# jonnydubowsky/hbbft

Measured on AMD Instinct MI355X. Metric: BLS12-381 share verifies/sec (node) at N=256; crypto ms per HB epoch, higher is better.
Workload: dtype i32 (Fq as 14 signed 28-bit digits, R = 2^392, in the share check; 12 x u32 limbs elsewhere)

## Files before the change

hbbft_amd/csrc/g1d.hpp:

```cpp
#pragma once
#include "g2d.hpp"

namespace hbx {

struct g1jd {
  fqd x, y, z;
};

HBX_HD g1jd g1d_dbl(const g1jd& p) {
  const fqd A = fqd_sqr(p.x);
  const fqd B = fqd_sqr(p.y);
  const fqd C = fqd_sqr(B);
  const fqd D = fqd_dbl(fqd_relax(fqd_sub(fqd_sub(fqd_sqr(fqd_add(p.x, B)), A), C)));
  const fqd E = fqd_relax(fqd_add(fqd_dbl(A), A));
  const fqd F = fqd_sqr(E);
  const fqd X3 = fqd_relax(fqd_sub(F, fqd_dbl(D)));
  const fqd C8 = fqd_dbl(fqd_dbl(fqd_dbl(C)));
  const fqd Y3 = fqd_relax(fqd_sub(fqd_mul(E, fqd_sub(D, X3)), C8));
  const fqd Z3 = fqd_relax(fqd_dbl(fqd_mul(p.y, p.z)));
  return g1jd{X3, Y3, Z3};
}

HBX_HD g1jd g1d_add_mixed(const g1jd& p, const fqd& qx, const fqd& qy) {
  const fqd one = fqd_const(FQD_ONE);
// ... 45 lines not shown
#pragma unroll 1
  for (int i = 2; i < 16; i++) tab[i] = g1d_add_mixed(tab[i - 1], px, py);
  const uint32_t top = k4[3] >> 28;
  g1jd acc = tab[top];
  bool ai = top == 0;
#pragma unroll 1
  for (int w = 30; w >= 0; w--) {
    const uint32_t nib = (k4[w >> 3] >> ((w & 7) * 4)) & 0xFu;
    if (!ai) {
#pragma unroll 1
      for (int q = 0; q < 4; q++) acc = g1d_dbl(acc);
    }
    if (nib) {
      acc = ai ? tab[nib] : g1d_add_nc(acc, tab[nib]);
      ai = false;
    }
  }
  if (ai) return g1_identity();
  return g1j{fqd_to_fq(acc.x), fqd_to_fq(acc.y), fqd_to_fq(acc.z)};
}

constexpr int G1D_TAB_N = 15;
constexpr int G1D_TABS = 2 * G1D_TAB_N;
HBX_HD uint32_t g1d_tab_stride(uint32_t form) { return form == 3 ? 1u : form == 0 ? (uint32_t)G1D_TAB_N : (uint32_t)G1D_TABS; }

HBX_HD void g1d_table15(const g1jd& P, g1jd* tab) {
  tab[0] = P;
  g1jd prev = P;
#pragma unroll 1
  for (int m = 2; m <= G1D_TAB_N; m++) {
    prev = (m & 1) ? g1d_add_nc(prev, P) : g1d_dbl(tab[m / 2 - 1]);
    tab[m - 1] = prev;
  }
}

HBX_HDNI void g1d_table15_ni(const g1jd& P, g1jd* tab) { g1d_table15(P, tab); }

HBX_HDNI void g1d_build_tables(const g1jd& S, g1jd* T, int parts) {
  g1jd d = S;
  if (parts & 6) {
#pragma unroll 1
    for (int i = 0; i < 64; i++) d = g1d_dbl(d);
  }
  if (parts & 4) T[0] = d;
#pragma unroll 1
  for (int h = 1; h >= 0; h--)
    if (parts & (1 << h)) g1d_table15(h ? d : S, T + (h ? 0 : G1D_TAB_N));
}

HBX_HDNI g1j g1d_mul_u128_tab(const g1jd* TS, const g1jd* TD, const uint32_t* k4, bool phi) {
  g1jd acc{fqd_const(FQD_ONE), fqd_const(FQD_ONE), fqd_zero()};
  bool ai = true;
#pragma unroll 1
  for (int w = 15; w >= 0; w--) {
    const uint32_t sh = (uint32_t)(w & 7) * 4;
    const uint32_t nl = (k4[w >> 3] >> sh) & 0xFu, nh = (k4[2 + (w >> 3)] >> sh) & 0xFu;
    const g1jd el = TS[nl ? nl - 1 : 0], eh = TD[nh ? nh - 1 : 0];
    if (!ai) {
#pragma unroll 1
      for (int q = 0; q < 4; q++) acc = g1d_dbl(acc);
    }
#pragma unroll 1
    for (int h = 0; h < 2; h++) {
      if (h ? nh : nl) {
        const g1jd& e = h ? eh : el;
        acc = ai ? e : g1d_add_nc(acc, e);
        ai = false;
      }
    }
  }
  if (ai) return g1_identity();
  if (phi) acc.x = fqd_mul(acc.x, fqd_from_fq(fq_from_const(G1_BETA)));
  return g1j{fqd_to_fq(acc.x), fqd_to_fq(acc.y), fqd_to_fq(acc.z)};
}

HBX_HDNI bool g1_is_torsion_free_d(const g1a& P) {
  if (P.inf) return true;
  const fqd px = fqd_from_fq(P.x), py = fqd_from_fq(P.y);
  g1jd acc{fqd_const(FQD_ONE), fqd_const(FQD_ONE), fqd_zero()};
#pragma unroll 1
  for (int i = 127; i >= 0; i--) {
    acc = g1d_dbl(acc);
    if ((G1_X2[i >> 5] >> (i & 31)) & 1) acc = g1d_add_mixed(acc, px, py);
  }
  if (fqd_is_zero_mod(acc.z)) return false;
  const fqd z2 = fqd_sqr(acc.z);
  const fqd z3 = fqd_mul(z2, acc.z);
  const fqd bx = fqd_mul(px, fqd_from_fq(fq_from_const(G1_BETA2)));
  return fqd_is_zero_mod(fqd_sub(acc.x, fqd_mul(bx, z2))) && fqd_is_zero_mod(fqd_add(acc.y, fqd_mul(py, z3)));
}

HBX_HDNI int32_t g1_decompress_d(const uint8_t* b48, g1a& out) {
  return g1_decompress_t(b48, out, [](const fq& a, fq& y) { return fq_sqrt_d(a, y); });
}

}
```

hbbft_amd/csrc/hbx_api.hip:

```cpp
#include <hip/hip_runtime.h>

#include <algorithm>
#include <atomic>
#include <cstdarg>
#include <cstdio>
#include <cstdlib>
#include <cstring>
#include <string>
#include <utility>
#include <vector>

#include "../../include/hbx.h"
#include "hbx_kernels.hip"
#include "broadcast.hpp"
#include "addplan.hpp"
#if defined(HBX_TU) && HBX_TU == 0
#include "_kdecl.hpp"
#endif

#if !defined(HBX_TU) || HBX_TU == 0
using namespace hbx;

namespace {

constexpr size_t FILL_WAVES = hbx_addplan::FILL_WAVES;
constexpr uint32_t COMB_FORM = 1;

std::atomic<uint64_t> live_buffers{0};

struct dbuf {
  void* p = nullptr;
  size_t cap = 0;
  dbuf() = default;
  dbuf(const dbuf&) = delete;
  dbuf& operator=(const dbuf&) = delete;
  ~dbuf() { release(); }
  bool ensure(size_t bytes) {
    if (bytes <= cap && p) return true;
    release();
    if (bytes == 0) bytes = 16;
    if (hipMalloc(&p, bytes) != hipSuccess) return false;
    live_buffers++;
    cap = bytes;
    return true;
  }
  void release() {
    if (p && hipFree(p) == hipSuccess) live_buffers--;
    p = nullptr;
    cap = 0;
// ... 90 lines not shown
  dbuf comb_partial, comb_done;
  dbuf pk, pk_m, pk64, pk_status, pk_comp;
  dbuf g1tab;
  uint32_t p_ct = 0;
  dbuf U, G2pts, Hj, lines, lines_d, scratch, ct_ok, ct_valid, dec_st;
  dbuf lines_u, line_degen;
  uint32_t own_me = UINT32_MAX;
  dbuf own_sk, own_S, own_part;
  bool own_ready = false;
  bool ct_known = false;
  const uint8_t* d_v_blob = nullptr;
  const uint64_t* d_v_off = nullptr;
  uint64_t max_v_len = 0;
  dbuf v_blob_own, v_off_own, u_comp_own, w_comp_own;
  uint32_t n_shares = 0, verified_p = 0;
  dbuf S, S_status, fallback, valid, shares_own, present_own, gslot;
  dbuf fe1slot;
  uint32_t verify_tiles = 0;
  dbuf add_S, add_status, add_valid, add_mask, add_zero, add_shares, add_dst;
  size_t add_mask_m = 0;
  uint32_t force_fallback = 0;
  uint32_t force_degen = 0;
  int32_t comb_margin = HBX_COMBINE_MARGIN_AUTO;
  dbuf comb_tab, comb_tab_ok, comb_slow;
  bool tab_ready = false;
  uint32_t comb_slow_p = 0;
  uint32_t tab_cap = 0, tab_me = UINT32_MAX, tab_n = 0, tab_p = 0, tab_form = 0;
  bool batch_on = false;
  uint64_t batch_call = 0;
  uint32_t batch_last_p = 0;
  dbuf b_seed, b_AJ, b_T, b_C, b_Asum, b_A, b_B, b_cls0, b_cand, b_pass, b_zero, b_cls, b_ctok, b_stats;
  dbuf fb_lanes, fb_coin, fb_ct, fb_sigs;
  dbuf* fb_last = nullptr;
  dbuf hs[6];
  dbuf keys, status, out_own;
  dbuf gf_log, gf_exp;
  uint32_t rs_k = 0, rs_m = 0;
  dbuf rs_enc, rs_enc_job, rs_enc_coef, rs_enc_ptab, rs_ptab_d, rs_ptab_p, rs_jobs_d, rs_jobs_p, rs_coef_d, rs_coef_p, leaf_hash, leaf_slots, val_digest, roots;
  dbuf rg_dev;
  pinbuf rg_pin;
  dev_event rg_ev;
  uint32_t coin_I = 0, coin_n = 0;
  dbuf coin_blob, coin_off, coin_H, coin_Hp, coin_lines, coin_scratch, coin_sk, coin_sig96, coin_sig, coin_sig_st, coin_present,
      coin_valid, coin_comb, coin_comb_st, coin_mpk_comp, coin_mpk, coin_mpk_st, coin_ok, coin_par, coin_out96;
  dbuf vs_pk, vs_blob, vs_off, vs_H, vs_lines, vs_lines_d, vs_scratch, vs_sig96, vs_sig, vs_sig_st, vs_status;
  dbuf vk_pk48, vk_pk, vk_pkst, vk_idx, vk_gslot, vk_sk;
  dbuf coin_lines_d;
// ... 576 lines not shown
  HIPCHK(c, hipMemcpyAsync(st.data(), c->pk_status.p, (size_t)n * 4, hipMemcpyDeviceToHost, c->stream));
  HIPCHK(c, hipStreamSynchronize(c->stream));
  if (status) memcpy(status, st.data(), (size_t)n * 4);
  c->n_keys = n;
  return HBX_OK;
}

int hbx_set_own_share(hbx_ctx* c, uint32_t me, const uint8_t* sk32) {
  if (!c) return HBX_E_INVALID_ARG;
  if (!sk32) {
    c->own_me = UINT32_MAX;
    c->own_ready = false;
    return HBX_OK;
  }
  if (c->n_keys == 0 || me >= c->n_keys) return fail(c, HBX_E_NO_KEYS, "hbx_set_own_share: me=%u, n=%u", me, c->n_keys);
  static const uint8_t ZERO[32] = {0};
  if (!scalars_canonical(sk32, 1) || memcmp(sk32, ZERO, 32) == 0)
    return fail(c, HBX_E_INVALID_ARG, "hbx_set_own_share: scalar must be in [1, r)");
  uint8_t pk48[48], want[48];
  int rc = hbx_public_keys(c, sk32, 1, pk48);
  if (rc) return rc;
  HIPCHK(c, hipMemcpy(want, static_cast<uint8_t*>(c->pk_comp.p) + (size_t)me * 48, 48, hipMemcpyDeviceToHost));
  if (memcmp(pk48, want, 48) != 0) return fail(c, HBX_E_INVALID_ARG, "hbx_set_own_share: sk does not match pk[%u]", me);
  uint32_t limbs[8];
  for (int q = 0; q < 8; q++)
    limbs[q] = ((uint32_t)sk32[31 - 4 * q - 3] << 24) | ((uint32_t)sk32[31 - 4 * q - 2] << 16) |
               ((uint32_t)sk32[31 - 4 * q - 1] << 8) | sk32[31 - 4 * q];
  if (!c->own_sk.ensure(32)) return fail(c, HBX_E_OUT_OF_MEMORY, "hbx_set_own_share: out of device memory");
  HIPCHK(c, quiesce(c));
  HIPCHK(c, hipMemcpy(c->own_sk.p, limbs, 32, hipMemcpyHostToDevice));
  c->own_me = me;
  c->own_ready = false;
  return HBX_OK;
}

static int launch_prepare_ct(hbx_ctx* c, hipStream_t s, const uint8_t* d_u_comp, const uint8_t* d_v_blob,
                             const uint64_t* d_v_off, const uint8_t* d_w_comp, uint32_t p, const uint8_t* early_shares,
                             size_t m_early, uint32_t early_n, uint32_t me_early) {
  const dim3 b64(64);
  const bool own = c->own_me != UINT32_MAX;
  {
    timed t_(c, HBX_K_PREPARE_CT, s);
    const uint32_t hash_blocks = (uint32_t)(((size_t)p * HASH_K + 63) / 64);
    const uint32_t dec_blocks = (own ? 4 : 2) * ((p + 63) / 64);
    const uint32_t share_blocks = (uint32_t)((m_early + 63) / 64);
    if (own && (!c->own_S.ensure((size_t)p * sizeof(g1a)) || !c->own_part.ensure((size_t)2 * p * sizeof(g1j))))
      return fail(c, HBX_E_OUT_OF_MEMORY, "hbx_prepare_ciphertexts_d: out of device memory");
    static const bool split = getenv("HBX_SPLIT_PREP") != nullptr;
    const uint32_t parts = split ? 2 : 1;
    for (uint32_t q = 0; q < parts; q++) {
      const uint32_t b0 = split && q == 1 ? hash_blocks : 0;
      const uint32_t nb = split ? (q == 0 ? hash_blocks : dec_blocks + share_blocks)
                                : hash_blocks + dec_blocks + share_blocks;
      hipLaunchKernelGGL(k_prepare_ct, dim3(nb), b64, 0, s, d_u_comp, d_v_blob, d_v_off, d_w_comp, p, hash_blocks,
                         c->U.as<g1a>(), c->G2pts.as<g2a>(), c->dec_st.as<int32_t>(),
                         own ? c->own_sk.as<uint32_t>() : nullptr, own ? c->own_part.as<g1j>() : nullptr, c->Hj.as<g2j>(), c->digest,
                         b0, dec_blocks, early_shares, m_early, early_n ? early_n : 1u, me_early, c->S.as<g1a>(),
                         c->S_status.as<int32_t>());
    }
    c->own_ready = own;
  }
  HIPCHK(c, hipGetLastError());
  return HBX_OK;
}

static int prepare_impl(hbx_ctx* c, const uint8_t* d_u_comp, const uint8_t* d_v_blob, const uint64_t* d_v_off,
                        const uint8_t* d_w_comp, uint32_t p, uint64_t max_v_len, uint8_t* d_ct_valid,
                        void* stream, const uint8_t* early_shares, uint32_t early_n, uint32_t tab_cap = 0) {
  if (!c || p == 0 || !d_u_comp || !d_v_off || !d_w_comp)
    return fail(c, HBX_E_INVALID_ARG, "hbx_prepare_ciphertexts_d: bad args");
  HBX_ENTER(c, stream);
  if (!c->U.ensure((size_t)p * sizeof(g1a)) || !c->G2pts.ensure((size_t)2 * p * sizeof(g2a)) || !c->Hj.ensure((size_t)p * sizeof(g2j)) ||
      !c->lines.ensure((size_t)p * sizeof(line_block)) || !c->lines_d.ensure((size_t)p * sizeof(line_block_d)) ||
      !c->lines_u.ensure((size_t)p * sizeof(line_block_d)) || !c->line_degen.ensure(p) ||
      !c->scratch.ensure((size_t)2 * p * MILLER_LINES * sizeof(fq2d)) || !c->ct_ok.ensure(p) ||
      !c->ct_valid.ensure(p) || !c->dec_st.ensure((size_t)2 * p * 4))
    return fail(c, HBX_E_OUT_OF_MEMORY, "hbx_prepare_ciphertexts_d: out of device memory");
  const size_t m_early = early_shares ? (size_t)early_n * p : 0;
  if (m_early && (!c->S.ensure(m_early * sizeof(g1a)) || !c->S_status.ensure(m_early * 4)))
    return fail(c, HBX_E_OUT_OF_MEMORY, "hbx_prepare_ciphertexts_d: out of device memory");
  static const char* form_env = getenv("HBX_COMB_FORM");
  const uint32_t form = form_env && form_env[0] >= '0' && form_env[0] <= '3' ? (uint32_t)(form_env[0] - '0') : COMB_FORM;
  c->tab_ready = false;
  if (!m_early) tab_cap = 0;
  if (tab_cap && (!c->comb_tab.ensure((size_t)p * (tab_cap + 1) * g1d_tab_stride(form) * sizeof(g1jd)) ||
                  !c->comb_tab_ok.ensure((size_t)p * (tab_cap + 1))))
    return fail(c, HBX_E_OUT_OF_MEMORY, "hbx_decrypt_epoch_d: out of device memory for the combine's tables");
  const dim3 b64(64);
  const bool own = c->own_me != UINT32_MAX;
  const uint32_t me_early = (own && c->own_me < early_n) ? c->own_me : UINT32_MAX;
  if (int rc = launch_prepare_ct(c, s, d_u_comp, d_v_blob, d_v_off, d_w_comp, p, early_shares, m_early, early_n, me_early))
    return rc;
  {
    timed t_(c, HBX_K_PREPARE_LINES, s);
    const uint32_t line_blocks = (2 * p * LINE_K + 63) / 64, own_blocks = own ? (p + 63) / 64 : 0;
    const bool own_entry = m_early && me_early != UINT32_MAX;
    const uint32_t tab_blocks =
        tab_cap ? (form == 2 ? 2 : 1) * ((own_entry ? own_blocks : 0) + (uint32_t)(((size_t)p * tab_cap + 63) / 64)) : 0;
    auto kpl = k_prepare_lines<true>;
    hipLaunchKernelGGL(kpl, dim3(line_blocks + own_blocks + tab_blocks), b64, 0, s, c->G2pts.as<g2a>(), 2 * p,
                       c->lines_d.as<line_pre_d>(), c->scratch.as<fq2d>(), c->dec_st.as<int32_t>(), p,
                       c->ct_ok.as<uint8_t>(), own ? c->own_part.as<g1j>() : nullptr,
                       own ? c->own_S.as<g1a>() : nullptr, early_n, me_early,
                       own_entry ? c->S.as<g1a>() : nullptr, own_entry ? c->S_status.as<int32_t>() : nullptr,
                       c->Hj.as<g2j>(), c->S.as<g1a>(), c->S_status.as<int32_t>(),
                       tab_cap ? c->comb_tab.as<g1jd>() : nullptr, c->comb_tab_ok.as<uint8_t>(), tab_cap, form);
    HIPCHK(c, hipGetLastError());
    const uint32_t nl = 2 * p * MILLER_LINES;
    HIPCHK(c, hipMemsetAsync(c->line_degen.p, 0, p, s));
    hipLaunchKernelGGL(k_normalise_lines, dim3((nl + 63) / 64), b64, 0, s, c->lines.as<line_pre>(),
                       c->scratch.as<fq2d>(), nl, c->lines_d.as<line_pre_d>(), c->G2pts.as<g2a>(),
                       c->Hj.as<g2j>(), c->lines_u.as<line_pre_d>(), c->line_degen.as<uint8_t>());
  }
  HIPCHK(c, hipGetLastError());
  c->p_ct = p;
  c->invalidate_epoch();
  c->tab_ready = tab_cap != 0;
  c->tab_cap = tab_cap;
  c->tab_me = me_early;
  c->tab_n = early_n;
  c->tab_p = p;
  c->tab_form = form;
  if (d_ct_valid) {
    if (!c->S.ensure(sizeof(g1a)) || !c->S_status.ensure(4) || !c->valid.ensure(16))
      return fail(c, HBX_E_OUT_OF_MEMORY, "hbx_prepare_ciphertexts_d: out of device memory");
    int rc = launch_pair_checks(c, s, 0, p, 0, 0, nullptr, c->ct_ok.as<uint8_t>());
    if (rc) return rc;
    HIPCHK(c, hipMemcpyAsync(d_ct_valid, c->ct_valid.p, p, hipMemcpyDeviceToDevice, s));
    c->ct_known = true;
// ... 867 lines not shown
  if (!c || !sk32 || !sig96 || n == 0) return fail(c, HBX_E_INVALID_ARG, "hbx_sign: bad args");
  if (c->coin_I == 0) return fail(c, HBX_E_NO_CIPHERTEXTS, "hbx_prepare_nonces has not been called");
  if (!scalars_canonical(sk32, n)) return fail(c, HBX_E_INVALID_ARG, "hbx_sign: scalar >= r");
  HBX_ENTER(c, c->stream);
  const size_t m = (size_t)n * c->coin_I;
  if (!c->coin_sk.ensure((size_t)n * 32) || !c->coin_sig96.ensure(m * 96))
    return fail(c, HBX_E_OUT_OF_MEMORY, "hbx_sign: out of device memory");
  HIPCHK(c, hipMemcpyAsync(c->coin_sk.p, sk32, (size_t)n * 32, hipMemcpyHostToDevice, s));
  if (int rc = coin_true_h(c, s)) return rc;
  hipLaunchKernelGGL(k_sign, dim3((n + 63) / 64, c->coin_I), dim3(64), 0, s, c->coin_sk.as<uint8_t>(), n,
                     c->coin_H.as<g2a>(), c->coin_sig96.as<uint8_t>());
  HIPCHK(c, hipGetLastError());
  HIPCHK(c, hipMemcpyAsync(sig96, c->coin_sig96.p, m * 96, hipMemcpyDeviceToHost, s));
  HIPCHK(c, hipStreamSynchronize(s));
  return HBX_OK;
}

static int coin_prepare_lines(hbx_ctx* c, hipStream_t s) {
  if (c->coin_lines_ready) return HBX_OK;
  const uint32_t count = c->coin_I;
  timed t_(c, HBX_K_PREPARE_LINES, s);
  hipLaunchKernelGGL(k_prepare_lines<true>, dim3((count * LINE_K + 63) / 64), dim3(64), 0, s, c->coin_Hp.as<g2a>(), count,
                     c->coin_lines_d.as<line_pre_d>(), c->coin_scratch.as<fq2d>(), nullptr, 0u, nullptr, nullptr, nullptr, 1u,
                     UINT32_MAX, nullptr, nullptr, nullptr, nullptr, nullptr, nullptr, nullptr, 0u, 0u);
  HIPCHK(c, hipGetLastError());
  const uint32_t nl = count * MILLER_LINES;
  hipLaunchKernelGGL(k_normalise_lines, dim3((nl + 63) / 64), dim3(64), 0, s, c->coin_lines.as<line_pre>(),
                     c->coin_scratch.as<fq2d>(), nl, c->coin_lines_d.as<line_pre_d>(), nullptr, nullptr, nullptr, nullptr);
  HIPCHK(c, hipGetLastError());
  c->coin_lines_ready = true;
  HIPCHK(c, c->coin_ready_ev.create());
  HIPCHK(c, hipEventRecord(c->coin_ready_ev.e, s));
  return HBX_OK;
}

static int launch_sig_checks(hbx_ctx* c, hipStream_t s, int lanes, dim3 grid, const uint2* tiles, const g2a* sig,
                             const int32_t* sig_st, const uint8_t* d_present, uint32_t n, uint8_t* vd) {
  timed t_(c, HBX_K_VERIFY_SIG, s);
  c->coin_lanes_used = lanes;
  c->coin_tiles = grid.x * grid.y;
  if (lanes == 2) {
    const size_t glanes = (size_t)grid.x * grid.y * 64;
    if (!c->gslot.ensure(glanes * 2 * LDS_FQ6D_PACKED * 4))
      return fail(c, HBX_E_OUT_OF_MEMORY, "hbx_verify_sig_shares: out of device memory (slots)");
    if (!c->fb_coin.ensure(4)) return fail(c, HBX_E_OUT_OF_MEMORY, "hbx_verify_sig_shares: out of device memory");
    HIPCHK(c, hipMemsetAsync(c->fb_coin.p, 0, 4, s));
    c->fb_last = &c->fb_coin;
// ... 95 lines not shown
  const uint64_t total = msg_off[count];
  if (total && !msg_blob) return fail(c, HBX_E_INVALID_ARG, "hbx_verify_sigs: null blob");
  HBX_ENTER(c, c->stream);
  if (!c->vs_pk.ensure((size_t)count * 48) || !c->vs_blob.ensure(total ? total : 16) ||
      !c->vs_off.ensure((size_t)(count + 1) * 8) || !c->vs_H.ensure((size_t)count * sizeof(g2a)) ||
      !c->vs_lines.ensure((size_t)count * MILLER_LINES * sizeof(line_pre)) ||
      !c->vs_lines_d.ensure((size_t)count * MILLER_LINES * sizeof(line_pre_d)) ||
      !c->vs_scratch.ensure((size_t)count * MILLER_LINES * sizeof(fq2d)) || !c->vs_sig96.ensure((size_t)count * 96) ||
      !c->vs_sig.ensure((size_t)count * sizeof(g2a)) || !c->vs_sig_st.ensure((size_t)count * 4) ||
      !c->vs_status.ensure(count))
    return fail(c, HBX_E_OUT_OF_MEMORY, "hbx_verify_sigs: out of device memory");
  HIPCHK(c, hipMemcpyAsync(c->vs_pk.p, pk48, (size_t)count * 48, hipMemcpyHostToDevice, s));
  if (total) HIPCHK(c, hipMemcpyAsync(c->vs_blob.p, msg_blob, total, hipMemcpyHostToDevice, s));
  HIPCHK(c, hipMemcpyAsync(c->vs_off.p, msg_off, (size_t)(count + 1) * 8, hipMemcpyHostToDevice, s));
  HIPCHK(c, hipMemcpyAsync(c->vs_sig96.p, sig96, (size_t)count * 96, hipMemcpyHostToDevice, s));
  hipLaunchKernelGGL(k_hash_nonces, dim3((unsigned)(((size_t)count * HASH_K + 63) / 64)), dim3(64), 0, s,
                     c->vs_blob.as<uint8_t>(), c->vs_off.as<uint64_t>(), count, c->vs_H.as<g2a>(), c->digest, 1);
  HIPCHK(c, hipGetLastError());
  hipLaunchKernelGGL(k_decompress_g2, dim3((count + 63) / 64), dim3(64), 0, s, c->vs_sig96.as<uint8_t>(), (size_t)count,
                     c->vs_sig.as<g2a>(), c->vs_sig_st.as<int32_t>(), 1u);
  HIPCHK(c, hipGetLastError());
  hipLaunchKernelGGL(k_prepare_lines<true>, dim3((count * LINE_K + 63) / 64), dim3(64), 0, s, c->vs_H.as<g2a>(), count,
                     c->vs_lines_d.as<line_pre_d>(), c->vs_scratch.as<fq2d>(), nullptr, 0u, nullptr, nullptr, nullptr, 1u,
                     UINT32_MAX, nullptr, nullptr, nullptr, nullptr, nullptr, nullptr, nullptr, 0u, 0u);
  HIPCHK(c, hipGetLastError());
  const uint32_t nl = count * MILLER_LINES;
  hipLaunchKernelGGL(k_normalise_lines, dim3((nl + 63) / 64), dim3(64), 0, s, c->vs_lines.as<line_pre>(),
                     c->vs_scratch.as<fq2d>(), nl, c->vs_lines_d.as<line_pre_d>(), nullptr, nullptr, nullptr, nullptr);
  HIPCHK(c, hipGetLastError());
  {
    timed t_(c, HBX_K_VERIFY_SIG, s);
    hipLaunchKernelGGL(k_verify_sigs, dim3((count + 63) / 64), dim3(64), 0, s, c->vs_pk.as<uint8_t>(),
                       c->vs_lines_d.as<line_pre_d>(), c->vs_H.as<g2a>(), c->vs_sig.as<g2a>(), c->vs_sig_st.as<int32_t>(),
                       count, c->vs_status.as<uint8_t>());
  }
  HIPCHK(c, hipGetLastError());
  HIPCHK(c, hipMemcpyAsync(status, c->vs_status.p, count, hipMemcpyDeviceToHost, s));
  HIPCHK(c, hipStreamSynchronize(s));
  return HBX_OK;
}

namespace {
constexpr uint32_t VERIFY_SIGS_CHUNK = 16384;

int msgs_check(hbx_ctx* c, const char* fn, const uint8_t* msg_blob, const uint64_t* msg_off, uint32_t count,
               uint64_t* total) {
  if (!msg_off || count == 0) return fail(c, HBX_E_INVALID_ARG, "%s: bad args", fn);
// ... 1112 lines not shown
```

hbbft_amd/csrc/hbx_kernels.hip:

```cpp
#include <hip/hip_runtime.h>
#include "../../include/hbx.h"
#include "hash.hpp"
#include "pairing.hpp"
#include "pairing3.hpp"
#include "pairingd.hpp"
#include "pairing3d.hpp"
#include "pairing2d.hpp"
#include "fe1d.hpp"
#include "g2d.hpp"
#include "g1d.hpp"
#include "curve4.hpp"
#include "wide.hpp"
#include "keygen.hpp"
#include "batchd.hpp"

#if !defined(HBX_TU)
#define HBX_IN_TU(n) 1
#else
#define HBX_IN_TU(n) (HBX_TU == (n))
#endif

namespace hbx {

struct line_block {
// ... 44 lines not shown
  if (i >= n) return;
  g1a p;
  const int32_t st = g1_decompress_d(comp + (size_t)i * 48, p);
  out[i] = p;
  status[i] = st;
}
#endif

constexpr int G1TAB_W = 64, G1TAB_D = 15;

constexpr int HASH_K = 16;

#if HBX_IN_TU(1)
__global__ void __launch_bounds__(64) k_prepare_ct(const uint8_t* __restrict__ u_comp,
                                                   const uint8_t* __restrict__ v_blob,
                                                   const uint64_t* __restrict__ v_off,
                                                   const uint8_t* __restrict__ w_comp, uint32_t p,
                                                   uint32_t hash_blocks, g1a* __restrict__ U,
                                                   g2a* __restrict__ G2pts, int32_t* __restrict__ dec_st,
                                                   const uint32_t* __restrict__ own_sk, g1j* __restrict__ own_part,
                                                   g2j* __restrict__ Hj, int digest, uint32_t block0, uint32_t dec_blocks,
                                                   const uint8_t* __restrict__ shares, size_t share_count,
                                                   uint32_t n, uint32_t me, g1a* __restrict__ S,
                                                   int32_t* __restrict__ S_status) {
  const uint32_t bid = blockIdx.x + block0;
  if (bid >= hash_blocks + dec_blocks) {
    const size_t i = (size_t)(bid - hash_blocks - dec_blocks) * blockDim.x + threadIdx.x;
    if (i >= share_count || (uint32_t)(i % n) == me) return;
    g1a q;
    int32_t st = g1_decompress_d(shares + i * 48, q);
    if (st == HBX_PT_OK && !g1_is_torsion_free_d(q)) st = HBX_PT_NOT_IN_SUBGROUP;
    S_status[i] = st;
    S[i] = q;
    return;
  }
  if (bid >= hash_blocks) {
    const uint32_t pw = (p + 63) & ~63u;
    const uint32_t k = (bid - hash_blocks) * blockDim.x + threadIdx.x;
    if (k < p) {
      g1a u;
      int32_t st = g1_decompress_d(u_comp + (size_t)k * 48, u);
      if (st == HBX_PT_OK && !g1_is_torsion_free_d(u)) st = HBX_PT_NOT_IN_SUBGROUP;
      dec_st[k] = st;
      U[k] = u;
    } else if (own_sk && k >= 2 * pw && k < 2 * pw + 2 * p) {
      const uint32_t h = k - 2 * pw, j = h >> 1;
      g1a u;
      g1j part = g1_identity();
      if (g1_decompress_d(u_comp + (size_t)j * 48, u) == HBX_PT_OK) {
        uint32_t k1[4], k2[4];
        g1_glv_split(own_sk, k1, k2);
        if (h & 1) u.x = fq_mul(u.x, fq_from_const(G1_BETA));
        part = g1_mul_u128(u, (h & 1) ? k2 : k1);
      }
      own_part[h] = part;
    } else if (k >= pw && k < pw + p) {
      const uint32_t j = k - pw;
      g2a w;
      int32_t st = g2_decompress(w_comp + (size_t)j * 96, w);
      if (st == HBX_PT_OK && !g2_is_torsion_free(w)) st = HBX_PT_NOT_IN_SUBGROUP;
      dec_st[p + j] = st;
      G2pts[2 * j + 1] = w;
    }
    return;
  }
  const uint32_t gid = bid * blockDim.x + threadIdx.x;
  const uint32_t j = gid / HASH_K;
  if (j >= p) return;
  const uint64_t off = v_off[j];
  const uint64_t len = v_off[j + 1] - off;
  uint8_t d[32];
  hash_g1_g2_digest(u_comp + (size_t)j * 48, v_blob + off, len, d, digest);
  g2j h;
  if (hash_g2_group<HASH_K>(d, true, h, false)) {
// ... 1 lines not shown
    g2a flag;
    flag.x = fq2_zero();
    flag.y = fq2_zero();
    flag.inf = g2j_is_identity(h);
    G2pts[2 * j] = flag;
  }
}
#endif

constexpr int LINE_K = 16;


#if HBX_IN_TU(1)
template <bool GADD>
__global__ void __launch_bounds__(64) k_prepare_lines(g2a* __restrict__ pts, uint32_t count,
                                                      line_pre_d* __restrict__ raw, fq2d* __restrict__ scratch,
                                                      const int32_t* __restrict__ dec_st, uint32_t p,
                                                      uint8_t* __restrict__ ct_ok, const g1j* __restrict__ own_part,
                                                      g1a* __restrict__ own_S, uint32_t n, uint32_t me,
                                                      g1a* __restrict__ S, int32_t* __restrict__ S_status,
                                                      const g2j* __restrict__ Hj, const g1a* __restrict__ tab_S,
                                                      const int32_t* __restrict__ tab_S_status,
                                                      g1jd* __restrict__ tabs, uint8_t* __restrict__ tab_ok,
                                                      uint32_t cap, uint32_t form) {
  const uint32_t line_blocks = (count * LINE_K + 63) / 64;
  if (blockIdx.x >= line_blocks) {
    uint32_t b = blockIdx.x - line_blocks;
    const uint32_t own_blocks = own_part ? (p + 63) / 64 : 0;
    if (b >= own_blocks) {
      if (!tabs) return;
      b -= own_blocks;
      const uint32_t slots = cap + 1;
      const uint32_t own_tab_blocks = (own_part && me != UINT32_MAX) ? own_blocks : 0;
      const uint32_t set_blocks = own_tab_blocks + (uint32_t)(((size_t)p * cap + 63) / 64);
      const bool second = b >= set_blocks;
      if (second) b -= set_blocks;
      const int parts = second ? 1 : form == 1 ? 3 : form == 3 ? 4 : 2;
      const uint32_t stride = g1d_tab_stride(form);
      if (b < own_tab_blocks) {
        const uint32_t j = b * blockDim.x + threadIdx.x;
        if (j >= p) return;
        const size_t slot = (size_t)j * slots + (me < cap ? me : cap);
        bool ok = false;
        if (dec_st[j] == HBX_PT_OK) {
          const g1j sum = g1_add(own_part[2 * j], own_part[2 * j + 1]);
          if (!g1j_is_identity(sum)) {
            g1d_build_tables(g1jd{fqd_from_fq(sum.x), fqd_from_fq(sum.y), fqd_from_fq(sum.z)}, tabs + slot * stride, parts);
            ok = true;
          }
        }
        if (!second) tab_ok[slot] = ok ? 1 : 0;
        return;
      }
      b -= own_tab_blocks;
      const size_t e = (size_t)b * blockDim.x + threadIdx.x;
      if (e >= (size_t)p * cap) return;
      const uint32_t j = (uint32_t)(e / cap), i = (uint32_t)(e % cap);
      if (i == me) return;
      const size_t slot = (size_t)j * slots + i;
      const g1a sp = tab_S[(size_t)j * n + i];
      const bool ok = tab_S_status[(size_t)j * n + i] == HBX_PT_OK && !sp.inf;
      if (ok) g1d_build_tables(g1jd{fqd_from_fq(sp.x), fqd_from_fq(sp.y), fqd_const(FQD_ONE)}, tabs + slot * stride, parts);
      if (!second) tab_ok[slot] = ok ? 1 : 0;
      return;
    }
    const uint32_t j = b * blockDim.x + threadIdx.x;
    if (j >= p) return;
    g1a sh;
    sh.x = fq_zero();
    sh.y = fq_zero();
    sh.inf = true;
    if (dec_st[j] == HBX_PT_OK) sh = g1_to_affine(g1_add(own_part[2 * j], own_part[2 * j + 1]));
    own_S[j] = sh;
    if (S) {
      S[(size_t)j * n + me] = sh;
      S_status[(size_t)j * n + me] = sh.inf ? HBX_PT_INFINITY : HBX_PT_OK;
    }
    return;
  }
  const uint32_t gid = blockIdx.x * blockDim.x + threadIdx.x;
  const uint32_t k = gid / LINE_K;
  const int gl = (int)(gid % LINE_K);
  if (k >= count) return;
  g2a q = pts[k];
  if (Hj && (k & 1) == 0) {
    q.x = Hj[k >> 1].x;
// ... 8 lines not shown
      if (!ok) {
        q.x = fq2_zero();
        q.y = fq2_zero();
        q.inf = true;
        if (gl == 0) pts[k] = q;
      }
    }
  }
  if (q.inf) {
    if (gl == 0) {
      const fq2d one{fqd_const(FQD_ONE), fqd_zero()}, zero{fqd_zero(), fqd_zero()};
      for (int i = 0; i < MILLER_LINES; i++) {
        raw[(size_t)k * MILLER_LINES + i] = line_pre_d{one, zero};
        scratch[(size_t)k * MILLER_LINES + i] = one;
      }
    }
    return;
  }
  g2d_raw_lines_group<GADD>(fq2d_from_fq2(q.x), fq2d_from_fq2(q.y), raw + (size_t)k * MILLER_LINES,
                            scratch + (size_t)k * MILLER_LINES, gl);
}
template __global__ void k_prepare_lines<true>(g2a*, uint32_t, line_pre_d*, fq2d*, const int32_t*, uint32_t, uint8_t*,
                                               const g1j*, g1a*, uint32_t, uint32_t, g1a*, int32_t*, const g2j*, const g1a*,
                                               const int32_t*, g1jd*, uint8_t*, uint32_t, uint32_t);
template __global__ void k_prepare_lines<false>(g2a*, uint32_t, line_pre_d*, fq2d*, const int32_t*, uint32_t, uint8_t*,
                                                const g1j*, g1a*, uint32_t, uint32_t, g1a*, int32_t*, const g2j*, const g1a*,
                                               const int32_t*, g1jd*, uint8_t*, uint32_t, uint32_t);

__global__ void __launch_bounds__(64) k_normalise_lines(line_pre* __restrict__ lines,
                                                        const fq2d* __restrict__ c2, uint32_t count,
                                                        line_pre_d* __restrict__ lines_d,
                                                        const g2a* __restrict__ pts, const g2j* __restrict__ Hj,
                                                        line_pre_d* __restrict__ lines_u,
                                                        uint8_t* __restrict__ degen) {
  const uint32_t k = blockIdx.x * blockDim.x + threadIdx.x;
  if (k >= count) return;
  const line_pre_d rd = lines_d[k];
  line_pre l{fq2d_to_fq2(rd.c0), fq2d_to_fq2(rd.c1)};
  const uint32_t pt = k / MILLER_LINES;
  fq2 z = fq2_one();
  if (Hj && (pt & 1) == 0 && !pts[pt].inf) z = Hj[pt >> 1].z;
  if (lines_u) {
    line_pre u;
    if (g2_normalise_line_z2(l, fq2d_to_fq2(c2[k]), z, u) && !pts[pt].inf) degen[pt >> 1] = 1;
    lines_u[k] = line_to_d(u);
  } else {
    g2_normalise_line_z(l, fq2d_to_fq2(c2[k]), z);
  }
  lines[k] = l;
  lines_d[k] = line_to_d(l);
// ... 480 lines not shown
    fr lam;
    if (lds_lag) {
      const fr xk = xm[k];
      const int h = q & 1, m0 = h ? (int)t / 2 : 0, m1 = h ? (int)t : (int)t / 2;
      fr den = h ? fr_from_const(FR_ONE) : xk;
      for (int m = m0; m < m1; m++)
        if (m != k) den = fr_mul(den, fr_sub(xm[m], xk));
      fr other;
#pragma unroll
      for (int w = 0; w < 8; w++) other.l[w] = (uint32_t)__shfl_xor((int)den.l[w], 1);
      den = fr_mul(den, other);
      lam = fr_from_mont(fr_mul(nall, fr_inv(den)));
    } else {
      lam = lagrange_at_zero(idx, (int)t, k);
    }
    uint32_t k1[4], k2[4];
    g1_glv_split(lam.l, k1, k2);
    const uint32_t i = idx[k];
    const uint32_t slot = i < cap ? i : (i == tab_me ? cap : UINT32_MAX);
    const size_t ts = (size_t)j * (cap + 1) + slot;
    g1a sp = S[(size_t)j * n + i];
    if (tabs && slot != UINT32_MAX && tab_ok[ts]) {
      const g1jd* T = tabs + ts * g1d_tab_stride(form);
      g1jd TS[G1D_TAB_N], TD[G1D_TAB_N];
      const bool have_s = form == 1 || form == 2, have_d = form != 3;
      if (!have_s) g1d_table15_ni(g1jd{fqd_from_fq(sp.x), fqd_from_fq(sp.y), fqd_const(FQD_ONE)}, TS);
      if (!have_d) g1d_table15_ni(T[0], TD);
      acc = g1_add(acc, g1d_mul_u128_tab(have_s ? T + G1D_TAB_N : TS, have_d ? T : TD, (q & 1) ? k2 : k1, (q & 1) != 0));
      continue;
    }
    atomicAdd(&slow_cnt, 1u);
    if (q & 1) sp.x = fq_mul(sp.x, fq_from_const(G1_BETA));
    acc = g1_add(acc, g1d_mul_u128_w4(sp, (q & 1) ? k2 : k1));
  }
  red[tid] = acc;
  __syncthreads();
  for (int stride = COMBINE_THREADS / 2; stride > 0; stride >>= 1) {
    if (tid < stride) red[tid] = g1_add(red[tid], red[tid + stride]);
    __syncthreads();
  }
  if (tid == 0) {
    slow[j] = slow_cnt;
    const g1a g = g1_to_affine(red[0]);
    uint8_t comp[48], d[32];
    g1_compress(g, comp);
    digest2(digest, comp, 48, nullptr, 0, d);
    for (int q = 0; q < 8; q++)
      keys[(size_t)j * 8 + q] = ((uint32_t)d[4 * q] << 24) | ((uint32_t)d[4 * q + 1] << 16) |
                                ((uint32_t)d[4 * q + 2] << 8) | d[4 * q + 3];
    status[j] = 0;
  }
// ... 1146 lines not shown
```

Baseline: 3.114 million.

## Use four-way comb tables for combine scalar multiplication, reusing torsion-check doublings

Switches the combine's default table form to four 15-entry windows spaced 32 doublings apart. Each 128-bit GLV half-scalar now needs 8 windows of 4 doublings instead of 16. The torsion check for shares is rewritten right-to-left so that its doubling chain stores the 2^32, 2^64 and 2^96 multiples, which then seed the extra tables without recomputing them. The host precomputes 2^32-shifted copies of the own secret key so the own-share partial products line up with the same tables. The cost is twice the table memory and bandwidth, more table-building threads, and a torsion check that now does a full add each step instead of a mixed add.

```diff
diff --git a/hbbft_amd/csrc/g1d.hpp b/hbbft_amd/csrc/g1d.hpp
--- a/hbbft_amd/csrc/g1d.hpp
+++ b/hbbft_amd/csrc/g1d.hpp
@@ -91,7 +91,8 @@
 
 constexpr int G1D_TAB_N = 15;
 constexpr int G1D_TABS = 2 * G1D_TAB_N;
-HBX_HD uint32_t g1d_tab_stride(uint32_t form) { return form == 3 ? 1u : form == 0 ? (uint32_t)G1D_TAB_N : (uint32_t)G1D_TABS; }
+constexpr int G1D_TABS4 = 4 * G1D_TAB_N;
+HBX_HD uint32_t g1d_tab_stride(uint32_t form) { return form == 4 ? (uint32_t)G1D_TABS4 : (uint32_t)G1D_TABS; }
 
 HBX_HD void g1d_table15(const g1jd& P, g1jd* tab) {
   tab[0] = P;
@@ -107,6 +108,17 @@
 
 HBX_HDNI void g1d_build_tables(const g1jd& S, g1jd* T, int parts) {
   g1jd d = S;
+  if (parts & 8) {
+#pragma unroll 1
+    for (int q = 0; q < 4; q++) {
+      if (q) {
+#pragma unroll 1
+        for (int i = 0; i < 32; i++) d = g1d_dbl(d);
+      }
+      g1d_table15(d, T + q * G1D_TAB_N);
+    }
+    return;
+  }
   if (parts & 6) {
 #pragma unroll 1
     for (int i = 0; i < 64; i++) d = g1d_dbl(d);
@@ -143,6 +155,37 @@
   return g1j{fqd_to_fq(acc.x), fqd_to_fq(acc.y), fqd_to_fq(acc.z)};
 }
 
+HBX_HDNI g1j g1d_mul_u128_tab4(const g1jd* T, const uint32_t* k4, bool phi) {
+  g1jd acc{fqd_const(FQD_ONE), fqd_const(FQD_ONE), fqd_zero()};
+  bool ai = true;
+#pragma unroll 1
+  for (int w = 7; w >= 0; w--) {
+    const uint32_t sh = (uint32_t)w * 4;
+    uint32_t nib = (k4[0] >> sh) & 0xFu;
+    g1jd next = T[nib ? nib - 1 : 0];
+    if (!ai) {
+#pragma unroll 1
+      for (int q = 0; q < 4; q++) acc = g1d_dbl(acc);
+    }
+#pragma unroll 1
+    for (int q = 0; q < 4; q++) {
+      const g1jd e = next;
+      const uint32_t n = nib;
+      if (q < 3) {
+        nib = (k4[q + 1] >> sh) & 0xFu;
+        next = T[(q + 1) * G1D_TAB_N + (nib ? nib - 1 : 0)];
+      }
+      if (n) {
+        acc = ai ? e : g1d_add_nc(acc, e);
+        ai = false;
+      }
+    }
+  }
+  if (ai) return g1_identity();
+  if (phi) acc.x = fqd_mul(acc.x, fqd_from_fq(fq_from_const(G1_BETA)));
+  return g1j{fqd_to_fq(acc.x), fqd_to_fq(acc.y), fqd_to_fq(acc.z)};
+}
+
 HBX_HDNI bool g1_is_torsion_free_d(const g1a& P) {
   if (P.inf) return true;
   const fqd px = fqd_from_fq(P.x), py = fqd_from_fq(P.y);
@@ -159,6 +202,55 @@
   return fqd_is_zero_mod(fqd_sub(acc.x, fqd_mul(bx, z2))) && fqd_is_zero_mod(fqd_add(acc.y, fqd_mul(py, z3)));
 }
 
+HBX_HD g1jd g1d_add_x(const g1jd& p, const g1jd& q, bool& inf) {
+  const fqd Z1Z1 = fqd_sqr(p.z);
+  const fqd Z2Z2 = fqd_sqr(q.z);
+  const fqd U1 = fqd_mul(p.x, Z2Z2);
+  const fqd U2 = fqd_mul(q.x, Z1Z1);
+  const fqd S1 = fqd_mul(fqd_mul(p.y, q.z), Z2Z2);
+  const fqd S2 = fqd_mul(fqd_mul(q.y, p.z), Z1Z1);
+  const fqd H = fqd_relax(fqd_sub(U2, U1));
+  const fqd rh = fqd_relax(fqd_sub(S2, S1));
+  if (fqd_is_zero_mod(H)) {
+    if (fqd_is_zero_mod(rh)) return g1d_dbl(p);
+    inf = true;
+    return p;
+  }
+  const fqd I = fqd_sqr(fqd_dbl(H));
+  const fqd J = fqd_mul(H, I);
+  const fqd r = fqd_dbl(rh);
+  const fqd V = fqd_mul(U1, I);
+  const fqd X3 = fqd_relax(fqd_sub(fqd_sub(fqd_sqr(r), J), fqd_dbl(V)));
+  const fqd Y3 = fqd_relax(fqd_sub(fqd_mul(r, fqd_sub(V, X3)), fqd_dbl(fqd_mul(S1, J))));
+  const fqd Z3 = fqd_mul(fqd_relax(fqd_sub(fqd_sub(fqd_sqr(fqd_relax(fqd_add(p.z, q.z))), Z1Z1), Z2Z2)), H);
+  return g1jd{X3, Y3, Z3};
+}
+
+HBX_HDNI bool g1_is_torsion_free_rl_d(const g1a& P, g1jd* D) {
+  const fqd px = fqd_from_fq(P.x), py = fqd_from_fq(P.y);
+  g1jd q{px, py, fqd_const(FQD_ONE)};
+  g1jd acc = q;
+  bool ai = true;
+#pragma unroll 1
+  for (int i = 0; i < 128; i++) {
+    if (i) q = g1d_dbl(q);
+    if (D && i && (i & 31) == 0) D[(i >> 5) - 1] = q;
+    if ((G1_X2[i >> 5] >> (i & 31)) & 1) {
+      if (ai) {
+        acc = q;
+        ai = false;
+      } else {
+        acc = g1d_add_x(acc, q, ai);
+      }
+    }
+  }
+  if (ai) return false;
+  const fqd z2 = fqd_sqr(acc.z);
+  const fqd z3 = fqd_mul(z2, acc.z);
+  const fqd bx = fqd_mul(px, fqd_from_fq(fq_from_const(G1_BETA2)));
+  return fqd_is_zero_mod(fqd_sub(acc.x, fqd_mul(bx, z2))) && fqd_is_zero_mod(fqd_add(acc.y, fqd_mul(py, z3)));
+}
+
 HBX_HDNI int32_t g1_decompress_d(const uint8_t* b48, g1a& out) {
   return g1_decompress_t(b48, out, [](const fq& a, fq& y) { return fq_sqrt_d(a, y); });
 }
diff --git a/hbbft_amd/csrc/hbx_api.hip b/hbbft_amd/csrc/hbx_api.hip
--- a/hbbft_amd/csrc/hbx_api.hip
+++ b/hbbft_amd/csrc/hbx_api.hip
@@ -24,7 +24,7 @@
 namespace {
 
 constexpr size_t FILL_WAVES = hbx_addplan::FILL_WAVES;
-constexpr uint32_t COMB_FORM = 1;
+constexpr uint32_t COMB_FORM = 4;
 
 std::atomic<uint64_t> live_buffers{0};
 
@@ -161,7 +161,7 @@
   uint32_t force_fallback = 0;
   uint32_t force_degen = 0;
   int32_t comb_margin = HBX_COMBINE_MARGIN_AUTO;
-  dbuf comb_tab, comb_tab_ok, comb_slow;
+  dbuf comb_tab, comb_tab_ok, comb_d, comb_slow;
   bool tab_ready = false;
   uint32_t comb_slow_p = 0;
   uint32_t tab_cap = 0, tab_me = UINT32_MAX, tab_n = 0, tab_p = 0, tab_form = 0;
@@ -784,13 +784,33 @@
   if (rc) return rc;
   HIPCHK(c, hipMemcpy(want, static_cast<uint8_t*>(c->pk_comp.p) + (size_t)me * 48, 48, hipMemcpyDeviceToHost));
   if (memcmp(pk48, want, 48) != 0) return fail(c, HBX_E_INVALID_ARG, "hbx_set_own_share: sk does not match pk[%u]", me);
-  uint32_t limbs[8];
+  uint32_t limbs[4][8];
   for (int q = 0; q < 8; q++)
-    limbs[q] = ((uint32_t)sk32[31 - 4 * q - 3] << 24) | ((uint32_t)sk32[31 - 4 * q - 2] << 16) |
-               ((uint32_t)sk32[31 - 4 * q - 1] << 8) | sk32[31 - 4 * q];
-  if (!c->own_sk.ensure(32)) return fail(c, HBX_E_OUT_OF_MEMORY, "hbx_set_own_share: out of device memory");
+    limbs[0][q] = ((uint32_t)sk32[31 - 4 * q - 3] << 24) | ((uint32_t)sk32[31 - 4 * q - 2] << 16) |
+                  ((uint32_t)sk32[31 - 4 * q - 1] << 8) | sk32[31 - 4 * q];
+  for (int q = 1; q < 4; q++) {
+    uint32_t* x = limbs[q];
+    memcpy(x, limbs[q - 1], 32);
+    for (int b = 0; b < 32; b++) {
+      for (int i = 7; i > 0; i--) x[i] = (x[i] << 1) | (x[i - 1] >> 31);
+      x[0] <<= 1;
+      bool ge = true;
+      for (int i = 7; i >= 0; i--)
+        if (x[i] != FR_R[i]) {
+          ge = x[i] > FR_R[i];
+          break;
+        }
+      uint64_t borrow = 0;
+      for (int i = 0; ge && i < 8; i++) {
+        const uint64_t d = (uint64_t)x[i] - FR_R[i] - borrow;
+        x[i] = (uint32_t)d;
+        borrow = (d >> 32) & 1;
+      }
+    }
+  }
+  if (!c->own_sk.ensure(sizeof limbs)) return fail(c, HBX_E_OUT_OF_MEMORY, "hbx_set_own_share: out of device memory");
   HIPCHK(c, quiesce(c));
-  HIPCHK(c, hipMemcpy(c->own_sk.p, limbs, 32, hipMemcpyHostToDevice));
+  HIPCHK(c, hipMemcpy(c->own_sk.p, limbs, sizeof limbs, hipMemcpyHostToDevice));
   c->own_me = me;
   c->own_ready = false;
   return HBX_OK;
@@ -798,15 +818,17 @@
 
 static int launch_prepare_ct(hbx_ctx* c, hipStream_t s, const uint8_t* d_u_comp, const uint8_t* d_v_blob,
                              const uint64_t* d_v_off, const uint8_t* d_w_comp, uint32_t p, const uint8_t* early_shares,
-                             size_t m_early, uint32_t early_n, uint32_t me_early) {
+                             size_t m_early, uint32_t early_n, uint32_t me_early, uint32_t tab_cap = 0,
+                             uint32_t tab_form = 0) {
   const dim3 b64(64);
   const bool own = c->own_me != UINT32_MAX;
   {
     timed t_(c, HBX_K_PREPARE_CT, s);
     const uint32_t hash_blocks = (uint32_t)(((size_t)p * HASH_K + 63) / 64);
-    const uint32_t dec_blocks = (own ? 4 : 2) * ((p + 63) / 64);
+    const uint32_t own_nq = !tab_cap ? 1u : tab_form == 4 ? 4u : 2u, own_qstep = tab_form == 4 ? 1u : 2u;
+    const uint32_t dec_blocks = (2 + (own ? 2 * own_nq : 0)) * ((p + 63) / 64);
     const uint32_t share_blocks = (uint32_t)((m_early + 63) / 64);
-    if (own && (!c->own_S.ensure((size_t)p * sizeof(g1a)) || !c->own_part.ensure((size_t)2 * p * sizeof(g1j))))
+    if (own && (!c->own_S.ensure((size_t)p * sizeof(g1a)) || !c->own_part.ensure((size_t)2 * p * own_nq * sizeof(g1j))))
       return fail(c, HBX_E_OUT_OF_MEMORY, "hbx_prepare_ciphertexts_d: out of device memory");
     static const bool split = getenv("HBX_SPLIT_PREP") != nullptr;
     const uint32_t parts = split ? 2 : 1;
@@ -818,7 +840,7 @@
                          c->U.as<g1a>(), c->G2pts.as<g2a>(), c->dec_st.as<int32_t>(),
                          own ? c->own_sk.as<uint32_t>() : nullptr, own ? c->own_part.as<g1j>() : nullptr, c->Hj.as<g2j>(), c->digest,
                          b0, dec_blocks, early_shares, m_early, early_n ? early_n : 1u, me_early, c->S.as<g1a>(),
-                         c->S_status.as<int32_t>());
+                         c->S_status.as<int32_t>(), own_nq, own_qstep, tab_cap ? c->comb_d.as<g1jd>() : nullptr, tab_cap);
     }
     c->own_ready = own;
   }
@@ -842,23 +864,26 @@
   if (m_early && (!c->S.ensure(m_early * sizeof(g1a)) || !c->S_status.ensure(m_early * 4)))
     return fail(c, HBX_E_OUT_OF_MEMORY, "hbx_prepare_ciphertexts_d: out of device memory");
   static const char* form_env = getenv("HBX_COMB_FORM");
-  const uint32_t form = form_env && form_env[0] >= '0' && form_env[0] <= '3' ? (uint32_t)(form_env[0] - '0') : COMB_FORM;
+  const uint32_t form = form_env && form_env[0] == '1' ? 1u : COMB_FORM;
   c->tab_ready = false;
   if (!m_early) tab_cap = 0;
   if (tab_cap && (!c->comb_tab.ensure((size_t)p * (tab_cap + 1) * g1d_tab_stride(form) * sizeof(g1jd)) ||
-                  !c->comb_tab_ok.ensure((size_t)p * (tab_cap + 1))))
+                  !c->comb_tab_ok.ensure((size_t)p * (tab_cap + 1)) ||
+                  !c->comb_d.ensure((size_t)p * (tab_cap + 1) * 3 * sizeof(g1jd))))
     return fail(c, HBX_E_OUT_OF_MEMORY, "hbx_decrypt_epoch_d: out of device memory for the combine's tables");
   const dim3 b64(64);
   const bool own = c->own_me != UINT32_MAX;
   const uint32_t me_early = (own && c->own_me < early_n) ? c->own_me : UINT32_MAX;
-  if (int rc = launch_prepare_ct(c, s, d_u_comp, d_v_blob, d_v_off, d_w_comp, p, early_shares, m_early, early_n, me_early))
+  if (int rc = launch_prepare_ct(c, s, d_u_comp, d_v_blob, d_v_off, d_w_comp, p, early_shares, m_early, early_n, me_early,
+                                 tab_cap, form))
     return rc;
   {
     timed t_(c, HBX_K_PREPARE_LINES, s);
     const uint32_t line_blocks = (2 * p * LINE_K + 63) / 64, own_blocks = own ? (p + 63) / 64 : 0;
     const bool own_entry = m_early && me_early != UINT32_MAX;
+    const uint32_t nq = form == 4 ? 4u : 2u;
     const uint32_t tab_blocks =
-        tab_cap ? (form == 2 ? 2 : 1) * ((own_entry ? own_blocks : 0) + (uint32_t)(((size_t)p * tab_cap + 63) / 64)) : 0;
+        tab_cap ? (own_entry ? (p * nq + 63) / 64 : 0) + (uint32_t)(((size_t)p * tab_cap * nq + 63) / 64) : 0;
     auto kpl = k_prepare_lines<true>;
     hipLaunchKernelGGL(kpl, dim3(line_blocks + own_blocks + tab_blocks), b64, 0, s, c->G2pts.as<g2a>(), 2 * p,
                        c->lines_d.as<line_pre_d>(), c->scratch.as<fq2d>(), c->dec_st.as<int32_t>(), p,
@@ -866,7 +891,8 @@
                        own ? c->own_S.as<g1a>() : nullptr, early_n, me_early,
                        own_entry ? c->S.as<g1a>() : nullptr, own_entry ? c->S_status.as<int32_t>() : nullptr,
                        c->Hj.as<g2j>(), c->S.as<g1a>(), c->S_status.as<int32_t>(),
-                       tab_cap ? c->comb_tab.as<g1jd>() : nullptr, c->comb_tab_ok.as<uint8_t>(), tab_cap, form);
+                       tab_cap ? c->comb_tab.as<g1jd>() : nullptr, c->comb_tab_ok.as<uint8_t>(), tab_cap, form,
+                       c->comb_d.as<g1jd>());
     HIPCHK(c, hipGetLastError());
     const uint32_t nl = 2 * p * MILLER_LINES;
     HIPCHK(c, hipMemsetAsync(c->line_degen.p, 0, p, s));
@@ -1780,7 +1806,7 @@
   timed t_(c, HBX_K_PREPARE_LINES, s);
   hipLaunchKernelGGL(k_prepare_lines<true>, dim3((count * LINE_K + 63) / 64), dim3(64), 0, s, c->coin_Hp.as<g2a>(), count,
                      c->coin_lines_d.as<line_pre_d>(), c->coin_scratch.as<fq2d>(), nullptr, 0u, nullptr, nullptr, nullptr, 1u,
-                     UINT32_MAX, nullptr, nullptr, nullptr, nullptr, nullptr, nullptr, nullptr, 0u, 0u);
+                     UINT32_MAX, nullptr, nullptr, nullptr, nullptr, nullptr, nullptr, nullptr, 0u, 0u, nullptr);
   HIPCHK(c, hipGetLastError());
   const uint32_t nl = count * MILLER_LINES;
   hipLaunchKernelGGL(k_normalise_lines, dim3((nl + 63) / 64), dim3(64), 0, s, c->coin_lines.as<line_pre>(),
@@ -1922,7 +1948,7 @@
   HIPCHK(c, hipGetLastError());
   hipLaunchKernelGGL(k_prepare_lines<true>, dim3((count * LINE_K + 63) / 64), dim3(64), 0, s, c->vs_H.as<g2a>(), count,
                      c->vs_lines_d.as<line_pre_d>(), c->vs_scratch.as<fq2d>(), nullptr, 0u, nullptr, nullptr, nullptr, 1u,
-                     UINT32_MAX, nullptr, nullptr, nullptr, nullptr, nullptr, nullptr, nullptr, 0u, 0u);
+                     UINT32_MAX, nullptr, nullptr, nullptr, nullptr, nullptr, nullptr, nullptr, 0u, 0u, nullptr);
   HIPCHK(c, hipGetLastError());
   const uint32_t nl = count * MILLER_LINES;
   hipLaunchKernelGGL(k_normalise_lines, dim3((nl + 63) / 64), dim3(64), 0, s, c->vs_lines.as<line_pre>(),
diff --git a/hbbft_amd/csrc/hbx_kernels.hip b/hbbft_amd/csrc/hbx_kernels.hip
--- a/hbbft_amd/csrc/hbx_kernels.hip
+++ b/hbbft_amd/csrc/hbx_kernels.hip
@@ -90,14 +90,20 @@
                                                    g2j* __restrict__ Hj, int digest, uint32_t block0, uint32_t dec_blocks,
                                                    const uint8_t* __restrict__ shares, size_t share_count,
                                                    uint32_t n, uint32_t me, g1a* __restrict__ S,
-                                                   int32_t* __restrict__ S_status) {
+                                                   int32_t* __restrict__ S_status, uint32_t own_nq,
+                                                   uint32_t own_qstep, g1jd* __restrict__ comb_d, uint32_t cap) {
   const uint32_t bid = blockIdx.x + block0;
   if (bid >= hash_blocks + dec_blocks) {
     const size_t i = (size_t)(bid - hash_blocks - dec_blocks) * blockDim.x + threadIdx.x;
     if (i >= share_count || (uint32_t)(i % n) == me) return;
     g1a q;
     int32_t st = g1_decompress_d(shares + i * 48, q);
-    if (st == HBX_PT_OK && !g1_is_torsion_free_d(q)) st = HBX_PT_NOT_IN_SUBGROUP;
+    if (st == HBX_PT_OK) {
+      const uint32_t sender = (uint32_t)(i % n);
+      const bool in_g1 = comb_d ? g1_is_torsion_free_rl_d(q, sender < cap ? comb_d + ((i / n) * (cap + 1) + sender) * 3 : nullptr)
+                                : g1_is_torsion_free_d(q);
+      if (!in_g1) st = HBX_PT_NOT_IN_SUBGROUP;
+    }
     S_status[i] = st;
     S[i] = q;
     return;
@@ -111,13 +117,13 @@
       if (st == HBX_PT_OK && !g1_is_torsion_free_d(u)) st = HBX_PT_NOT_IN_SUBGROUP;
       dec_st[k] = st;
       U[k] = u;
-    } else if (own_sk && k >= 2 * pw && k < 2 * pw + 2 * p) {
-      const uint32_t h = k - 2 * pw, j = h >> 1;
+    } else if (own_sk && k >= 2 * pw && k < 2 * pw + 2 * p * own_nq) {
+      const uint32_t h = k - 2 * pw, q = own_nq > 1 ? h / (2 * p) : 0, j = (h - q * 2 * p) >> 1;
       g1a u;
       g1j part = g1_identity();
       if (g1_decompress_d(u_comp + (size_t)j * 48, u) == HBX_PT_OK) {
         uint32_t k1[4], k2[4];
-        g1_glv_split(own_sk, k1, k2);
+        g1_glv_split(own_sk + 8 * q * own_qstep, k1, k2);
         if (h & 1) u.x = fq_mul(u.x, fq_from_const(G1_BETA));
         part = g1_mul_u128(u, (h & 1) ? k2 : k1);
       }
@@ -165,7 +171,8 @@
                                                       const g2j* __restrict__ Hj, const g1a* __restrict__ tab_S,
                                                       const int32_t* __restrict__ tab_S_status,
                                                       g1jd* __restrict__ tabs, uint8_t* __restrict__ tab_ok,
-                                                      uint32_t cap, uint32_t form) {
+                                                      uint32_t cap, uint32_t form,
+                                                      const g1jd* __restrict__ comb_d) {
   const uint32_t line_blocks = (count * LINE_K + 63) / 64;
   if (blockIdx.x >= line_blocks) {
     uint32_t b = blockIdx.x - line_blocks;
@@ -173,38 +180,38 @@
     if (b >= own_blocks) {
       if (!tabs) return;
       b -= own_blocks;
-      const uint32_t slots = cap + 1;
-      const uint32_t own_tab_blocks = (own_part && me != UINT32_MAX) ? own_blocks : 0;
-      const uint32_t set_blocks = own_tab_blocks + (uint32_t)(((size_t)p * cap + 63) / 64);
-      const bool second = b >= set_blocks;
-      if (second) b -= set_blocks;
-      const int parts = second ? 1 : form == 1 ? 3 : form == 3 ? 4 : 2;
+      const uint32_t slots = cap + 1, nq = form == 4 ? 4u : 2u, qstep = form == 4 ? 1u : 2u;
+      const uint32_t own_tab_blocks = (own_part && me != UINT32_MAX) ? (p * nq + 63) / 64 : 0;
       const uint32_t stride = g1d_tab_stride(form);
       if (b < own_tab_blocks) {
-        const uint32_t j = b * blockDim.x + threadIdx.x;
-        if (j >= p) return;
+        const uint32_t e = b * blockDim.x + threadIdx.x;
+        if (e >= p * nq) return;
+        const uint32_t j = e / nq, q = e % nq;
         const size_t slot = (size_t)j * slots + (me < cap ? me : cap);
         bool ok = false;
         if (dec_st[j] == HBX_PT_OK) {
-          const g1j sum = g1_add(own_part[2 * j], own_part[2 * j + 1]);
+          const g1j sum = g1_add(own_part[(size_t)2 * p * q + 2 * j], own_part[(size_t)2 * p * q + 2 * j + 1]);
           if (!g1j_is_identity(sum)) {
-            g1d_build_tables(g1jd{fqd_from_fq(sum.x), fqd_from_fq(sum.y), fqd_from_fq(sum.z)}, tabs + slot * stride, parts);
+            g1d_table15(g1jd{fqd_from_fq(sum.x), fqd_from_fq(sum.y), fqd_from_fq(sum.z)},
+                        tabs + slot * stride + q * G1D_TAB_N);
             ok = true;
           }
         }
-        if (!second) tab_ok[slot] = ok ? 1 : 0;
+        if (q == 0) tab_ok[slot] = ok ? 1 : 0;
         return;
       }
       b -= own_tab_blocks;
       const size_t e = (size_t)b * blockDim.x + threadIdx.x;
-      if (e >= (size_t)p * cap) return;
-      const uint32_t j = (uint32_t)(e / cap), i = (uint32_t)(e % cap);
+      if (e >= (size_t)p * cap * nq) return;
+      const uint32_t q = (uint32_t)(e % nq), i = (uint32_t)(e / nq % cap), j = (uint32_t)(e / nq / cap);
       if (i == me) return;
       const size_t slot = (size_t)j * slots + i;
       const g1a sp = tab_S[(size_t)j * n + i];
       const bool ok = tab_S_status[(size_t)j * n + i] == HBX_PT_OK && !sp.inf;
-      if (ok) g1d_build_tables(g1jd{fqd_from_fq(sp.x), fqd_from_fq(sp.y), fqd_const(FQD_ONE)}, tabs + slot * stride, parts);
-      if (!second) tab_ok[slot] = ok ? 1 : 0;
+      if (ok)
+        g1d_table15(q ? comb_d[slot * 3 + q * qstep - 1] : g1jd{fqd_from_fq(sp.x), fqd_from_fq(sp.y), fqd_const(FQD_ONE)},
+                    tabs + slot * stride + q * G1D_TAB_N);
+      if (q == 0) tab_ok[slot] = ok ? 1 : 0;
       return;
     }
     const uint32_t j = b * blockDim.x + threadIdx.x;
@@ -259,10 +266,10 @@
 }
 template __global__ void k_prepare_lines<true>(g2a*, uint32_t, line_pre_d*, fq2d*, const int32_t*, uint32_t, uint8_t*,
                                                const g1j*, g1a*, uint32_t, uint32_t, g1a*, int32_t*, const g2j*, const g1a*,
-                                               const int32_t*, g1jd*, uint8_t*, uint32_t, uint32_t);
+                                               const int32_t*, g1jd*, uint8_t*, uint32_t, uint32_t, const g1jd*);
 template __global__ void k_prepare_lines<false>(g2a*, uint32_t, line_pre_d*, fq2d*, const int32_t*, uint32_t, uint8_t*,
                                                 const g1j*, g1a*, uint32_t, uint32_t, g1a*, int32_t*, const g2j*, const g1a*,
-                                               const int32_t*, g1jd*, uint8_t*, uint32_t, uint32_t);
+                                               const int32_t*, g1jd*, uint8_t*, uint32_t, uint32_t, const g1jd*);
 
 __global__ void __launch_bounds__(64) k_normalise_lines(line_pre* __restrict__ lines,
                                                         const fq2d* __restrict__ c2, uint32_t count,
@@ -789,11 +796,8 @@
     g1a sp = S[(size_t)j * n + i];
     if (tabs && slot != UINT32_MAX && tab_ok[ts]) {
       const g1jd* T = tabs + ts * g1d_tab_stride(form);
-      g1jd TS[G1D_TAB_N], TD[G1D_TAB_N];
-      const bool have_s = form == 1 || form == 2, have_d = form != 3;
-      if (!have_s) g1d_table15_ni(g1jd{fqd_from_fq(sp.x), fqd_from_fq(sp.y), fqd_const(FQD_ONE)}, TS);
-      if (!have_d) g1d_table15_ni(T[0], TD);
-      acc = g1_add(acc, g1d_mul_u128_tab(have_s ? T + G1D_TAB_N : TS, have_d ? T : TD, (q & 1) ? k2 : k1, (q & 1) != 0));
+      acc = g1_add(acc, form == 4 ? g1d_mul_u128_tab4(T, (q & 1) ? k2 : k1, (q & 1) != 0)
+                                  : g1d_mul_u128_tab(T, T + G1D_TAB_N, (q & 1) ? k2 : k1, (q & 1) != 0));
       continue;
     }
     atomicAdd(&slow_cnt, 1u);
```

After: 3.121 million, median of 6. Within noise of the previous version (+0.2%).
